# EavianWoo/SinGS

Hardware: AMD Instinct MI355X
Metric: rendered views/sec fwd+bwd, 200k Gaussians @1080p (higher is better)
Workload: dtype f32; 1 GPU; S(200000,1920,1080,deg=3,seed=3): 200000 Gaussians, 1920x1080, SH deg 3, fwd+bwd, R=780064 (tile,Gaussian) pairs, every view of a step within 0.1 % of that (cameras a few cm apart), frame-parallel dp1; gaussians=200000, width=1920, height=1080, sh_degree=3, num_rendered=780064, tile_list_max=135, frames_per_launch=8, streams=2, regularisers=False, forward_only=False, hip_graph=False, reduction=fold of 2 gradient row(s) for 16 views + collective in 1 chunk(s), gradient_rows=2, parallelism=dp1

## Files before the change

### sings_amd/_lib.py

```python
import ctypes as C
import os

_HERE = os.path.dirname(os.path.abspath(__file__))
LIB_PATH = os.environ.get("SINGS_HIP_LIB") or os.path.join(_HERE, "libsings_hip.so")
_lib = None


class SgRasterSettings(C.Structure):
    _fields_ = [
        ("image_height", C.c_int32), ("image_width", C.c_int32),
        ("tanfovx", C.c_float), ("tanfovy", C.c_float), ("scale_modifier", C.c_float),
        ("sh_degree", C.c_int32), ("sh_coeffs", C.c_int32),
        ("prefiltered", C.c_int32), ("debug", C.c_int32), ("flags", C.c_int32),
        ("bg", C.c_void_p), ("viewmatrix", C.c_void_p), ("projmatrix", C.c_void_p), ("campos", C.c_void_p),
        ("count_signal", C.c_void_p), ("count_signal_host", C.c_void_p),
    ]


class SgLayout(C.Structure):
    _fields_ = [(n, C.c_size_t) for n in (
        "geom_recA", "geom_recB", "geom_recC", "geom_depth", "geom_flags", "geom_slot", "geom_bytes",
        "bin_header", "bin_tile_count", "bin_ranges", "bin_cursor", "bin_pair_keys", "bin_point_list",
        "bin_point_keys", "bin_pair_gid", "bin_pair_tile", "bin_pair_local", "bin_sort_items", "bin_rank_items", "bin_items", "bin_ck_start", "bin_plan", "bin_pair_mask", "bin_item_w", "bin_item_perm", "bin_rec_valid", "bin_tile_keys", "bin_bytes", "img_final_T", "img_n_contrib", "img_ckpt", "img_bytes", "bwd_bytes")]


class SgSkinInputs(C.Structure):
    _fields_ = [("J", C.c_int32), ("rot_format", C.c_int32)] + [(n, C.c_void_p) for n in (
        "xyz_canon", "rot_canon", "lbs_weights", "A", "smpl_scale", "transl", "ext_trans", "ext_rot", "ext_scale")]
# ... 115 lines not shown
    "sg_mesh_midpoints_i32": "i: i3 p4",
    "sg_mesh_collapse_max_edges": "i:",
    "sg_mesh_collapse_ws_bytes": "z: i2",
    "sg_mesh_collapse_build": "i: i3 p3 d p3",
    "sg_mesh_collapse_emit": "i: i4 p6",
    "sg_init_ws_bytes": "z: i",
    "sg_init_attributes": "i: i3 f2 p12",
    "sg_attr_mse_ws_bytes": "z:",
    "sg_attr_mse": "i: i V3 p3",
    "sg_plateau_step": "i: i3 d p4 i p i p",
    "sg_profile_enable": "i: i",
    "sg_copy_probe": "i: p2 z i p",
    "sg_profile_collect": "i: d n i",
    "sg_kernel_name": "s: i",
}
_PROTOTYPES_EVAL = {
    "sg_image_metrics_ws_bytes": "z: i3",
    "sg_image_metrics_frames": "i: i4 p2 z p z p3",
}
_PROTOTYPES_MESH_TERMS = {
    "sg_mesh_terms_build": "i: i3 p13",
    "sg_mesh_terms": "i: i p4 i p13",
}
_P = C.POINTER
_CTYPE = {"i": C.c_int, "z": C.c_size_t, "f": C.c_float, "s": C.c_char_p,
          "p": C.c_void_p,
          "S": _P(SgRasterSettings), "F": _P(SgFrameBatch), "K": _P(SgSkinInputs), "L": _P(SgLayout), "T": _P(SgTriplane),
          "D": _P(SgLinearSide),
          "n": _P(C.c_int64), "Z": _P(C.c_size_t), "d": _P(C.c_double),
          "V": _P(C.c_void_p),
          "G": _P(C.c_void_p * 3 * 4)}
EXPORTS = tuple(_PROTOTYPES)
LPIPS_NUM_OFFSETS = 46
LPIPS_WS_NUM_PIECES = 28
LPIPS_MIN_SIZE = 16
NUM_KERNELS = 8
ABI_VERSION = 8
METRICS_CLAMP = 1
METRICS_FLOATS = 8
METRICS_STRIP_COLS = 64
METRICS_CHUNK_ROWS = 32
MESH_TERMS_INFO_INTS = 2
MESH_TERMS_BAD_LABEL = 1
MESH_TERMS_BAD_EDGE = 2
FLAG_SHORT_LISTS = 1
COUNT_FLAG_HALF_ROWS = 4
COUNT_FLAG_HALF_LONG_ROWS = 8
FLAG_WS_CLEAN = 2
FLAG_THROUGHPUT = 4
FLAG_FORWARD_BINNING = 8
FLAG_FORWARD_COMPOSITE = 16
FLAG_SH_PLANAR = 32
FLAG_LONG_ROWS = 64
NUM_RENDERED_LONG_LIST = -2
HDR_FLAG_OVERFLOW = 1
HDR_FLAG_LONG_LIST = 2


def _ctypes_of(signature):
    ret, _, params = signature.partition(":")
    return _CTYPE[ret], [_CTYPE[t[0]] for t in params.split() for _ in range(int(t[1:] or 1))]


def load():
    global _lib
    if _lib is not None:
        return _lib
    if not os.path.exists(LIB_PATH):
        raise RuntimeError(
            f"sings_amd: HIP library not built ({LIB_PATH} missing). There is no CPU fallback; "
            "run `make -C sings_amd/csrc` (needs hipcc, --offload-arch=gfx950).")
    import torch
    lib = C.CDLL(LIB_PATH)
    if lib.sg_abi_version() != ABI_VERSION:
        raise RuntimeError(f"sings_amd: {LIB_PATH} speaks ABI {lib.sg_abi_version()}, this host code ABI {ABI_VERSION} "
                           "(include/sings_hip.h SG_ABI_VERSION): rebuild with `make -C sings_amd/csrc`")
    for name, signature in (*_PROTOTYPES.items(), *_PROTOTYPES_EVAL.items(), *_PROTOTYPES_MESH_TERMS.items()):
        fn = getattr(lib, name)
        fn.restype, fn.argtypes = _ctypes_of(signature)
    _lib = lib
    return lib


def check(status, what):
    if status != 0:
        raise RuntimeError(f"sings_hip {what} failed: {load().sg_last_error().decode()}")


def layout(P, W, H, cap):
    L = SgLayout()
    check(load().sg_layout(P, W, H, cap, C.byref(L)), "sg_layout")
    return L


def aux_layout(P, W, H, cap):
    n = C.c_size_t(0)
    check(load().sg_aux_layout(P, W, H, cap, C.byref(n)), "sg_aux_layout")
    return int(n.value)


# ... 5 lines not shown
```

### sings_amd/csrc/sg_api_raster.hip

```cpp
#include "sg_host.h"

#include <chrono>
#include <stdlib.h>
#include <thread>

static int sg_make_cam(const SgRasterSettings *s, SgCam *c)
{
    if (!s || s->image_width <= 0 || s->image_height <= 0 || !s->viewmatrix || !s->projmatrix || !s->campos || !s->bg)
        return 1;
    if (s->sh_degree < 0 || s->sh_degree > 3) return 1;
    c->W = s->image_width; c->H = s->image_height;
    c->gx = (c->W + SG_TILE - 1) / SG_TILE; c->gy = (c->H + SG_TILE - 1) / SG_TILE;
    if ((size_t)c->gx * (size_t)c->gy >= SG_MAX_TILES) return 1;
    c->tanfovx = s->tanfovx; c->tanfovy = s->tanfovy;
    c->fx = (float)c->W / (2.0f * s->tanfovx); c->fy = (float)c->H / (2.0f * s->tanfovy);
    c->mod = s->scale_modifier; c->D = s->sh_degree; c->M = s->sh_coeffs; c->flags = s->flags;
    c->view = s->viewmatrix; c->proj = s->projmatrix; c->campos = s->campos; c->bg = s->bg;
    c->count_signal = nullptr;
    return 0;
}

static void sg_arm_count(const SgRasterSettings *s, SgCam *c, const int64_t *num_rendered_host)
{
    if (!num_rendered_host || !s->count_signal || !s->count_signal_host) return;
// ... 85 lines not shown
    hipError_t e = hipMemcpy2DAsync(r, 8, binning_ws, bin_stride ? bin_stride : 8, 8, (size_t)K, hipMemcpyDeviceToHost, (hipStream_t)stream);
    if (e == hipSuccess) e = hipStreamSynchronize((hipStream_t)stream);
    if (e != hipSuccess) return sg_set_error("sg_read_num_rendered", e);
    for (int f = 0; f < K; f++)
        num_rendered_host[f] = (r[2 * f + 1] & 2u) ? (int64_t)SG_NUM_RENDERED_LONG_LIST : (int64_t)r[2 * f];
    return 0;
}

enum SgAux { SG_AUX_NONE, SG_AUX_ONE, SG_AUX_FRAMES };

static int sg_aux_flags(const char *who, int flags, bool frames)
{
    static const struct { int bit; const char *name; } refused[] = {
        { SG_FLAG_THROUGHPUT, "SG_FLAG_THROUGHPUT" }, { SG_FLAG_FORWARD_BINNING, "SG_FLAG_FORWARD_BINNING" },
        { SG_FLAG_FORWARD_COMPOSITE, "SG_FLAG_FORWARD_COMPOSITE" }, { SG_FLAG_SH_PLANAR, "SG_FLAG_SH_PLANAR" } };
    for (const auto &r : refused)
        if ((flags & r.bit) && !(frames && r.bit == SG_FLAG_THROUGHPUT))
            return sg_failf("%s: %s is not supported with depth / alpha maps", who, r.name);
    const int known = SG_FLAG_SHORT_LISTS | SG_FLAG_LONG_ROWS | SG_FLAG_WS_CLEAN | (frames ? SG_FLAG_THROUGHPUT : 0);
    if (flags & ~known) return sg_failf("%s: unknown flags 0x%x", who, flags & ~known);
    return 0;
}

static int sg_forward_impl(const char *who, const SgRasterSettings *s, const SgFrameBatch *fb, int P, const SgSkinInputs *skin,
                           const float *means3D, const float *shs, const float *colors_precomp, const float *opacities,
                           const float *scales, const float *rotations, const float *cov3D_precomp, void *geom_ws, void *binning_ws,
                           size_t cap, void *image_ws, float *out_color, int32_t *radii, float *posed_xyz, float *posed_rotq,
                           float *posed_scales, int write_point_keys, int64_t *num_rendered_host, void *stream,
                           SgAux aux = SG_AUX_NONE, void *aux_ws = nullptr, float *out_depth = nullptr, float *out_alpha = nullptr)
{
    hipStream_t st = (hipStream_t)stream;
    SgCam c;
    if (aux && !aux_ws) return sg_failf("%s: null pointer (aux_ws)", who);
    if (sg_make_cam(s, &c)) return sg_failf("%s: bad settings", who);
    if (aux) {
        if (sg_aux_flags(who, c.flags, aux == SG_AUX_FRAMES)) return 1;
        if (!out_depth || !out_alpha) return sg_failf("%s: null pointer (out_depth / out_alpha)", who);
    }
    if (skin) {
        if (sg_check_skin(skin, P, true)) return sg_failf("%s: bad skin inputs (J in 1..64, ext_tfs all or none)", who);
        if (sg_check_placement(who, fb, skin)) return 1;
        if (P < 0 || !geom_ws || !binning_ws || !image_ws || !out_color || (P > 0 && (!shs || !opacities || !scales || !radii)))
            return sg_failf("%s: null pointer", who);
        if (s->sh_coeffs < (s->sh_degree + 1) * (s->sh_degree + 1)) return sg_failf("%s: sh_coeffs smaller than (sh_degree+1)^2", who);
    } else {
        if (sg_check_placement(who, fb, nullptr)) return 1;
        if (P < 0 || !geom_ws || !binning_ws || !image_ws || !out_color || (P > 0 && (!means3D || !opacities || !radii)))
            return sg_failf("%s: null pointer", who);
        if (P > 0 && ((shs != nullptr) == (colors_precomp != nullptr))) return sg_failf("%s: provide exactly one of shs / colors_precomp", who);
        if (P > 0 && (((scales != nullptr) && (rotations != nullptr)) == (cov3D_precomp != nullptr)))
            return sg_failf("%s: provide exactly one of (scales,rotations) / cov3D_precomp", who);
        if (shs && (s->sh_coeffs < (s->sh_degree + 1) * (s->sh_degree + 1))) return sg_failf("%s: sh_coeffs smaller than (sh_degree+1)^2", who);
    }
    SgLayout L;
    sg_layout(P, c.W, c.H, cap, &L);
    SgBatch bt;
    if (sg_make_batch(fb, P, c, L, cap, &bt)) return sg_failf("%s: bad frame batch (K in 1..16, camera_stride 0|1, transl_stride 0|3)", who);
    SgGeom g = sg_geom_view(geom_ws, L);
    SgBin b = sg_bin_view(binning_ws, L);
    SgImg im = sg_img_view(image_ws, L);
    const bool do_bin = !(c.flags & SG_FLAG_FORWARD_COMPOSITE), do_comp = !(c.flags & SG_FLAG_FORWARD_BINNING);
    if (!do_bin && !do_comp) return sg_failf("%s: SG_FLAG_FORWARD_BINNING and SG_FLAG_FORWARD_COMPOSITE exclude each other", who);
    if (do_bin) {
        if (bt.K == 1) sg_arm_count(s, &c, num_rendered_host);
        if (!(c.flags & SG_FLAG_WS_CLEAN)) {
            const size_t zb = (L.bin_tile_count - L.bin_header) + sg_ctr_count((uint32_t)c.gx, (uint32_t)c.gy) * 4;
            for (int f = 0; f < bt.K; f++) sg_zero_async((char *)b.header + (size_t)f * bt.bin, zb, st);
        }
        if (skin) sg_launch_skin_fwd(c, bt, P, skin, shs, opacities, scales, g, b, cap, radii, posed_xyz, posed_rotq, posed_scales, st);
        else sg_launch_preprocess_fwd(c, bt, P, means3D, shs, colors_precomp, opacities, scales, rotations, cov3D_precomp, g, b, cap, radii, st);
        SG_CHECK_LAST("preprocess_fwd", s, st);
        sg_launch_binning(c, bt, P, radii, g, b, cap, write_point_keys, st);
        SG_CHECK_LAST("binning", s, st);
    }
    if (do_comp) {
        SgAuxFwd ax = sg_aux_fwd_view(aux_ws, g, out_depth, out_alpha);
        ax.ws = sg_aux_bytes(cap); ax.map = (size_t)c.W * (size_t)c.H;
        sg_launch_render_fwd(c, bt, g, b, cap, im, out_color, write_point_keys, st, aux ? &ax : nullptr);
        SG_CHECK_LAST("render_fwd", s, st);
    }
    if (!do_bin) return 0;
    if (bt.K == 1) return sg_finish_count(s, c, binning_ws, num_rendered_host, stream);
    return num_rendered_host ? sg_read_counts(binning_ws, bt.bin, bt.K, num_rendered_host, stream) : 0;
}

extern "C" int sg_rasterize_forward(const SgRasterSettings *s, int P, const float *means3D, const float *shs,
                                    const float *colors_precomp, const float *opacities, const float *scales,
                                    const float *rotations, const float *cov3D_precomp, void *geom_ws,
                                    void *binning_ws, size_t cap, void *image_ws, float *out_color,
                                    int32_t *radii, int write_point_keys, int64_t *num_rendered_host, void *stream)
{
    return sg_forward_impl("sg_rasterize_forward", s, &SG_ONE_FRAME, P, nullptr, means3D, shs, colors_precomp, opacities, scales,
                           rotations, cov3D_precomp, geom_ws, binning_ws, cap, image_ws, out_color, radii, nullptr, nullptr, nullptr,
// ... 355 lines not shown
extern "C" int sg_rasterize_backward_records_frames_aux(const SgRasterSettings *s, const SgFrameBatch *fb, int P, const void *geom_ws,
                                                        const void *binning_ws, size_t cap, const void *image_ws, void *bwd_ws,
                                                        const float *dL_dout_color, void *aux_ws, const float *dL_ddepth,
                                                        const float *dL_dalpha, void *stream)
{
    return sg_records_impl("sg_rasterize_backward_records_frames_aux", s, fb, P, geom_ws, binning_ws, cap, image_ws, bwd_ws,
                           dL_dout_color, stream, SG_AUX_FRAMES, aux_ws, dL_ddepth, dL_dalpha);
}

extern "C" int sg_skinned_backward_gaussians_frames_aux(const SgRasterSettings *s, const SgFrameBatch *fb, int P, const SgSkinInputs *skin,
                                                        const float *shs, const float *opacities, const float *scales,
                                                        const int32_t *radii, const void *geom_ws, const void *binning_ws, size_t cap,
                                                        const void *bwd_ws, float *skin_ws, int accumulate,
                                                        const float *dL_dposed_xyz_in, const float *dL_dposed_rotq_in,
                                                        float *dL_dxyz_canon, float *dL_drot_canon, float *dL_dscales,
                                                        float *dL_dopacity, float *dL_dsh, float *dL_dmeans2D, float *dL_dA,
                                                        float *dL_dtransl, void *aux_ws, void *stream)
{
    (void)opacities;
    return sg_skin_gaussians_impl("sg_skinned_backward_gaussians_frames_aux", s, fb, P, skin, shs, scales, radii, geom_ws, binning_ws,
                                  cap, bwd_ws, skin_ws, accumulate, dL_dposed_xyz_in, dL_dposed_rotq_in, dL_dxyz_canon, dL_drot_canon,
                                  dL_dscales, dL_dopacity, dL_dsh, dL_dmeans2D, dL_dA, dL_dtransl, stream, SG_AUX_FRAMES, aux_ws);
}
```

### sings_amd/csrc/sg_host.h

```cpp
#pragma once
#include "sg_common.h"

#include <math.h>
#include <stdarg.h>
#include <stdio.h>

static inline int sg_failf(const char *fmt, ...)
{
    char msg[256];
    va_list ap;
    va_start(ap, fmt);
    vsnprintf(msg, sizeof msg, fmt, ap);
    va_end(ap);
    return sg_set_error(msg, hipSuccess);
}

static inline int sg_launched(const char *what)
{
    const hipError_t e = hipGetLastError();
    return e == hipSuccess ? 0 : sg_set_error(what, e);
}

static inline void sg_ssim_window(float w[11])
{
    float g[11];
    double s = 0.0;
    for (int x = 0; x < 11; x++) { g[x] = (float)exp(-(double)((x - 5) * (x - 5)) / (2.0 * 1.5 * 1.5)); s += (double)g[x]; }
    for (int x = 0; x < 11; x++) w[x] = g[x] / (float)s;
}

#define SG_CHECK_LAST(what, s, st)                                           \
    do {                                                                     \
        hipError_t e_ = hipGetLastError();                                   \
        if (e_ != hipSuccess) return sg_set_error(what, e_);                 \
        if ((s)->debug) {                                                    \
            e_ = hipStreamSynchronize(st);                                   \
            if (e_ != hipSuccess) return sg_set_error(what, e_);             \
        }                                                                    \
    } while (0)

int sg_launch_linear_bwd_fan(int N, int Cin, int Cout, int act, const float *z, const float *dh, const float *W, float *dz_out,
                             float *dx_out, const SgLinearSide *side, hipStream_t st);
void sg_launch_scales_head(int N, const float *z, float *scales, float *aux, const float *dscales, const float *daux, float *dz,
                           hipStream_t st);
void sg_launch_rows_laplacian(int R, int V, int C, const float *x, const int *row_ptr, const int *col, const float *val,
                              const float *rscale, const int *t_row_ptr, const int *t_row, const float *t_val, void *ws, float *g_ws,
                              float *loss, const float *upstream, float *dL_dx, hipStream_t st);
```

### sings_amd/csrc/sg_preprocess.hip

```cpp
#include "sg_project.h"

template <int D>
__global__ void __launch_bounds__(256)
sg_preprocess_fwd_kernel(SgCam c, SgBatch bt, int P, const float *__restrict__ means3D,
                         const float *__restrict__ shs, const float *__restrict__ colors_precomp,
                         const float *__restrict__ opacities, const float *__restrict__ scales,
                         const float *__restrict__ rotations, const float *__restrict__ cov3D_precomp,
                         SgGeom g, SgBin bn, uint32_t cap, int32_t *__restrict__ radii, int hist_tiles, int nblocks)
{
    extern __shared__ uint32_t sg_hist_lds[];
    __shared__ uint32_t scratch_all[4][256];
    int gblock, frame;
    if (!sg_block_frame((int)blockIdx.x, bt.K, nblocks, gblock, frame)) return;
    c = sg_frame(c, frame, bt.cam_stride); g = sg_frame(g, (size_t)frame * bt.geom); bn = sg_frame(bn, (size_t)frame * bt.bin);
    radii += (size_t)frame * bt.P;
    const int idx = gblock * 256 + (int)threadIdx.x;
    const int wave = threadIdx.x >> 6;
    const bool live = idx < P;
    constexpr int nc = (D + 1) * (D + 1);
    float sh[nc * 3];
    if (shs && live) {
        const float *src = shs + (size_t)idx * c.M * 3;
        if (D == 3 && c.M == 16) {
#pragma unroll
            for (int k = 0; k < nc * 3 / 4; k++) {
                const float4 v = ((const float4 *)src)[k];
                sh[4 * k] = v.x; sh[4 * k + 1] = v.y; sh[4 * k + 2] = v.z; sh[4 * k + 3] = v.w;
            }
        } else {
#pragma unroll
            for (int k = 0; k < nc * 3; k++) sh[k] = src[k];
        }
    }
    SgProj o;
    o.mr = 0; o.tt = 0; o.clampbits = 0; o.x0 = o.y0 = o.x1 = o.y1 = 0;
    o.pix[0] = o.pix[1] = 0; o.conic[0] = o.conic[1] = o.conic[2] = 0; o.rgb[0] = o.rgb[1] = o.rgb[2] = 0; o.depth = 0;
    float opac = 0.0f;
    if (live) {
        float p[3] = { means3D[3 * idx], means3D[3 * idx + 1], means3D[3 * idx + 2] };
        float s3[3] = { 0, 0, 0 }, q[4] = { 0, 0, 0, 0 };
        if (!cov3D_precomp) {
            s3[0] = scales[3 * idx]; s3[1] = scales[3 * idx + 1]; s3[2] = scales[3 * idx + 2];
            q[0] = rotations[4 * idx]; q[1] = rotations[4 * idx + 1]; q[2] = rotations[4 * idx + 2]; q[3] = rotations[4 * idx + 3];
        }
        sg_project_fwd<D>(c, p, s3, q, cov3D_precomp ? cov3D_precomp + 6 * (size_t)idx : nullptr,
                          colors_precomp ? colors_precomp + 3 * (size_t)idx : nullptr, sh, o);
        opac = opacities[idx];
    }
    sg_store_proj(live, idx, o, opac, g, bn, c.gx, cap, radii, scratch_all[wave], hist_tiles ? sg_hist_lds : nullptr, hist_tiles,
                  sg_key_pitch_of(hist_tiles != 0, c.flags));
}

void sg_launch_preprocess_fwd(const SgCam &c, const SgBatch &bt, int P, const float *means3D, const float *shs,
                              const float *colors_precomp, const float *opacities, const float *scales,
                              const float *rotations, const float *cov3D_precomp, SgGeom g, SgBin b,
                              size_t cap, int32_t *radii, hipStream_t st)
{
    if (P <= 0) return;
    const int nblocks = (P + 255) / 256;
    dim3 grid(sg_frame_grid(nblocks, bt.K)), block(256);
    const int ht = sg_lds_hist(c.gx, c.gy) ? (int)sg_ctr_count((uint32_t)c.gx, (uint32_t)c.gy) : 0;
#define SG_PP(DD) hipLaunchKernelGGL(sg_preprocess_fwd_kernel<DD>, grid, block, (size_t)ht * 4, st, c, bt, P, means3D, shs, \
                                     colors_precomp, opacities, scales, rotations, cov3D_precomp, g, b, sg_cap32(cap), radii, ht, nblocks)
    int D = colors_precomp ? 0 : c.D;
    sg_prof_begin(SG_K_PREPROCESS_FWD, st);
    switch (D) { case 0: SG_PP(0); break; case 1: SG_PP(1); break; case 2: SG_PP(2); break; default: SG_PP(3); break; }
    sg_prof_end(SG_K_PREPROCESS_FWD, st);
#undef SG_PP
}

#define SG_PBWD_PARAMS SgCam c, int P, const float *__restrict__ means3D, const float *__restrict__ shs,                              \
                       const float *__restrict__ colors_precomp, const float *__restrict__ scales,                                \
                       const float *__restrict__ rotations, const float *__restrict__ cov3D_precomp,                              \
                       const int32_t *__restrict__ radii, SgGeom g, SgRec grec,                                                   \
                       size_t cap, const uint32_t *__restrict__ header, const uint8_t *__restrict__ rec_valid, float *__restrict__ dL_dmeans3D, float *__restrict__ dL_dmeans2D, \
                       float *__restrict__ dL_dsh, float *__restrict__ dL_dcolors,                                                \
                       float *__restrict__ dL_dopacity, float *__restrict__ dL_dscales,                                           \
                       float *__restrict__ dL_drots, float *__restrict__ dL_dcov3D
#define SG_PBWD_AUX 0
#include "sg_preprocess_bwd.inc"
#undef SG_PBWD_AUX
#define SG_PBWD_AUX 1
#include "sg_preprocess_bwd.inc"
#undef SG_PBWD_AUX

#define SG_ACC_PITCH 257
template <int D, bool ACC>
__global__ void __launch_bounds__(256) __attribute__((amdgpu_waves_per_eu(2, D >= 2 ? 2 : 3)))
sg_preprocess_bwd_frames_kernel(SgCam c0, SgBatch bt, int P, const float *__restrict__ means3D, const float *__restrict__ shs,
                         const float *__restrict__ colors_precomp, const float *__restrict__ scales,
                         const float *__restrict__ rotations, const float *__restrict__ cov3D_precomp,
// ... 231 lines not shown
```

### sings_amd/csrc/sg_project.h

```cpp
#pragma once
#include "sg_math.h"

template <int D>
__device__ __forceinline__ void sg_eval_sh(const float *__restrict__ sh, const float dir[3],
                                           float rgb[3], uint32_t &clampbits)
{
    float b[16];
    sg_sh_basis<D>(dir, b);
    constexpr int nc = (D + 1) * (D + 1);
    clampbits = 0;
#pragma unroll
    for (int c = 0; c < 3; c++) {
        float acc = b[0] * sh[c];
#pragma unroll
        for (int k = 1; k < nc; k++) acc = acc + b[k] * sh[3 * k + c];
        acc = acc + 0.5f;
        if (acc < 0.0f) { clampbits |= 1u << c; acc = 0.0f; }
        rgb[c] = acc;
    }
}


struct SgProj {
    int mr;
// ... 178 lines not shown
        }
    }
    if (expand) {
#pragma unroll
        for (int u = 0; u < 4; u++) {
            const uint32_t p = 64 * u + lane;
            const uint32_t slot = base + p;
            if (direct) {
                if (p < total) {
                    const uint32_t rank = local0[u] + (hist ? hist[ctr0[u]] : 0u);
                    if (rank < key_pitch) SG_KEY_STORE(&bn.tile_keys[(size_t)tile0[u] * key_pitch + rank], ((uint64_t)dep0[u] << 32) | gj0[u]);
                    else bn.header[8] = 1u;
                    if (hist && slot < cap) bn.rec_valid[slot] = 0;
                }
            } else if (p < total && slot < cap) {
                bn.pair_gid[slot] = gj0[u]; bn.pair_tile[slot] = tile0[u];
                bn.pair_local[slot] = local0[u] + (hist ? hist[ctr0[u]] : 0u);
            }
        }
    }
    __builtin_amdgcn_wave_barrier();
}

#define SG_ROW_LDS 52
__device__ __forceinline__ void sg_rows48_load(const float *__restrict__ base, int g0, int P, int lane,
                                               float *__restrict__ l)
{
    const float4 *src = (const float4 *)(base + (size_t)g0 * 48);
    const int nf4 = (P - g0 < 64 ? P - g0 : 64) * 12;
#pragma unroll
    for (int i = 0; i < 12; i++) {
        const int f = i * 64 + lane;
        if (f < nf4) {
            const float4 v = src[f];
            const int row = f / 12, c4 = f - row * 12;
            *(float4 *)(l + row * SG_ROW_LDS + 4 * c4) = v;
        }
    }
}
__device__ __forceinline__ void sg_rows48_store(float *__restrict__ base, int g0, int P, int lane,
                                                const float *__restrict__ l, int rows = 64, bool accumulate = false)
{
    float4 *dst = (float4 *)(base + (size_t)g0 * 48);
    const int nf4 = (P - g0 < rows ? (P - g0 > 0 ? P - g0 : 0) : rows) * 12;
    if (accumulate) {
        float4 old[12];
// ... 290 lines not shown
```

### sings_amd/engine.py

```python
import ctypes as C

import torch

from . import _lib
from ._marshal import _camera_stride, _frame_batch, _frame_rows, _ptr, _settings_struct, _skin_frames, _skin_struct
from ._marshal import _stream as _current_stream


def _raster_fields(M):
    return [("d_means3D", 3), ("d_scales", 3), ("d_rots", 4), ("d_opacity", 1), ("d_sh", 3 * M if M else None)]


def _skinned_fields(M, with_rot, rot_width):
    return [("d_xyz", 3), ("d_scales", 3), ("d_opacity", 1), ("d_sh", 3 * M), ("d_rot", int(rot_width) if with_rot else None)]


class _Engine:

    def __init__(self, P, W, H, sh_coeffs, device, capacity_pairs, K=None):
        self.lib = _lib.load()
        if K is not None and not 1 <= K <= _lib.MAX_FRAMES:
            raise ValueError(f"K must be 1..{_lib.MAX_FRAMES}")
        self.P, self.W, self.H, self.M, self.cap = int(P), int(W), int(H), int(sh_coeffs), int(capacity_pairs)
        self.K = 1 if K is None else int(K)
        self.dev = torch.device(device)
        L = _lib.SgLayout()
        sizes = [C.c_size_t() for _ in range(4)]
        _lib.check(self.lib.sg_frames_layout(self.P, self.W, self.H, self.cap, self.K, C.byref(L), *[C.byref(x) for x in sizes]),
                   "sg_frames_layout")
# ... 355 lines not shown
                       "skinned backward (records, frames, depth / alpha maps)")
        else:
            _lib.check(self.lib.sg_rasterize_backward_records_frames(*args, self._stream()), "skinned backward (records, frames)")

    def backward_gaussians(self, shs, opacities, scales, accumulate=False):
        self._check_backward()
        accumulate, done = self._chain_begin(accumulate)
        if self.aux and accumulate:
            raise ValueError("SkinnedFramesEngine: the depth / alpha maps (aux=True) write the gradients (no accumulate)")
        args = (C.byref(self._s), C.byref(self._fb), self.P, C.byref(self._k), _ptr(shs), _ptr(opacities), _ptr(scales),
                _ptr(self.radii), _ptr(self.geom), _ptr(self.binning), self.cap, _ptr(self.bwd_ws), _ptr(self.skin_ws),
                int(accumulate), None, None, _ptr(self.d_xyz), _ptr(self.d_rot), _ptr(self.d_scales), _ptr(self.d_opacity),
                _ptr(self.d_sh), _ptr(self.d_means2D), _ptr(self.d_A), _ptr(self.d_transl))
        if self.aux:
            _lib.check(self.lib.sg_skinned_backward_gaussians_frames_aux(*args, _ptr(self.aux_ws), self._stream()),
                       "skinned backward (gaussians, frames, depth / alpha maps)")
        else:
            _lib.check(self.lib.sg_skinned_backward_gaussians_frames(*args, self._stream()), "skinned backward (gaussians, frames)")
        self._chain_end(done)


class RasterFramesEngine(_FramesEngine):

    def __init__(self, P, W, H, sh_coeffs, K, device, capacity_pairs, grad_flat=None, sh_planar=False):
        super().__init__(P, W, H, sh_coeffs, device, capacity_pairs, K)
        self._gradients(_raster_fields(self.M), grad_flat, sh_planar)

    def set_camera(self, raster_settings, short_lists=False, long_rows=False):
        self._camera(raster_settings, (_lib.FLAG_SHORT_LISTS if short_lists else 0) | (_lib.FLAG_LONG_ROWS if long_rows else 0))
        self._fb = _frame_batch(self.K, self._cam_stride, 0)

    def forward(self, means3D, shs, opacities, scales, rotations, sync_num_rendered=False):
        if self._s is None or self._fb is None:
            raise RuntimeError("RasterFramesEngine: set_camera() first")
        nr = (C.c_int64 * self.K)()
        self._s.flags = self._flags()
        self._clean = False
        _lib.check(self.lib.sg_rasterize_forward_frames(
            C.byref(self._s), C.byref(self._fb), self.P, _ptr(means3D), _ptr(shs), None, _ptr(opacities), _ptr(scales),
            _ptr(rotations), None, _ptr(self.geom), _ptr(self.binning), self.cap, _ptr(self.img), _ptr(self.color),
            _ptr(self.radii), nr if sync_num_rendered else None, self._stream()), "forward (frames)")
        self._clean = True
        return [int(v) for v in nr] if sync_num_rendered else None

    def backward(self, means3D, shs, opacities, scales, rotations, dL_dcolor, accumulate=False):
        _lib.check(self.lib.sg_rasterize_backward_records_frames(
            C.byref(self._s), C.byref(self._fb), self.P, _ptr(self.geom), _ptr(self.binning), self.cap, _ptr(self.img),
            _ptr(self.bwd_ws), _ptr(dL_dcolor), self._stream()), "backward (records, frames)")
        accumulate, done = self._chain_begin(accumulate)
        _lib.check(self.lib.sg_rasterize_backward_gaussians_frames(
            C.byref(self._s), C.byref(self._fb), self.P, _ptr(means3D), _ptr(shs), None, _ptr(opacities), _ptr(scales),
            _ptr(rotations), None, _ptr(self.radii), _ptr(self.geom), _ptr(self.binning), self.cap, _ptr(self.bwd_ws),
            int(accumulate), _ptr(self.d_means3D), _ptr(self.d_means2D), _ptr(self.d_sh), None, _ptr(self.d_opacity),
            _ptr(self.d_scales), _ptr(self.d_rots), None, self._stream()), "backward (gaussians, frames)")
        self._chain_end(done)


class FramePipeline:

    def __init__(self, engines, device):
        self.engines = list(engines)
        self.dev = torch.device(device)
        self.A = torch.cuda.Stream(self.dev)
        self.B = torch.cuda.Stream(self.dev, priority=-1)
# ... 35 lines not shown
```

Baseline: 5473 views/s.

## Bin Gaussians in Morton work order with windowed LDS tile counting

Computes 3D Morton codes of the Gaussian means on the GPU, sorts them once into a work order, and splits forward preprocessing into a no-binning projection kernel plus an ordered binning kernel. The binning kernel visits Gaussians in spatial order so each block's tile footprint is compact and can be counted in an LDS window before global atomics. The goal is fewer contended global atomics on tile counters when the per-tile histogram does not fit in LDS. It costs an extra kernel launch and an order built once and cached, which can go stale as the Gaussians move.

```diff
diff --git a/include/sings_order.h b/include/sings_order.h
--- /dev/null
+++ b/include/sings_order.h
@@ -0,0 +1,26 @@
+#ifndef SINGS_ORDER_H
+#define SINGS_ORDER_H
+
+#include "sings_hip.h"
+
+#ifdef __cplusplus
+extern "C" {
+#endif
+
+#define SG_ORDER_WINDOW_TILES 1536
+#define SG_ORDER_BLOCK 256
+#define SG_ORDER_CODE_BITS 10
+#define SG_ORDER_WS_BYTES 32
+
+int sg_rasterize_forward_frames_ordered(const SgRasterSettings *s, const SgFrameBatch *fb, int P, const float *means3D,
+                                        const float *shs, const float *colors_precomp, const float *opacities,
+                                        const float *scales, const float *rotations, const float *cov3D_precomp, void *geom_ws,
+                                        void *binning_ws, size_t cap, void *image_ws, float *out_color, int32_t *radii,
+                                        int64_t *num_rendered_host, const uint32_t *order, int order_len, void *stream);
+
+int sg_work_order_codes(int P, const float *means3D, void *ws, uint32_t *codes, void *stream);
+
+#ifdef __cplusplus
+}
+#endif
+#endif
diff --git a/sings_amd/_lib.py b/sings_amd/_lib.py
--- a/sings_amd/_lib.py
+++ b/sings_amd/_lib.py
@@ -4,6 +4,7 @@
 _HERE = os.path.dirname(os.path.abspath(__file__))
 LIB_PATH = os.environ.get("SINGS_HIP_LIB") or os.path.join(_HERE, "libsings_hip.so")
 _lib = None
+HAS_ORDER = False
 
 
 class SgRasterSettings(C.Structure):
@@ -165,6 +166,10 @@
     "sg_mesh_terms_build": "i: i3 p13",
     "sg_mesh_terms": "i: i p4 i p13",
 }
+_PROTOTYPES_ORDER = {
+    "sg_rasterize_forward_frames_ordered": "i: S F i p9 z p3 n p i p",
+    "sg_work_order_codes": "i: i p4",
+}
 _P = C.POINTER
 _CTYPE = {"i": C.c_int, "z": C.c_size_t, "f": C.c_float, "s": C.c_char_p,
           "p": C.c_void_p,
@@ -183,6 +188,11 @@
 METRICS_FLOATS = 8
 METRICS_STRIP_COLS = 64
 METRICS_CHUNK_ROWS = 32
+ORDER_WINDOW_TILES = 1536
+ORDER_BLOCK = 256
+ORDER_CODE_BITS = 10
+ORDER_WS_BYTES = 32
+HIST_TILES_MAX = 4096
 MESH_TERMS_INFO_INTS = 2
 MESH_TERMS_BAD_LABEL = 1
 MESH_TERMS_BAD_EDGE = 2
@@ -218,7 +228,12 @@
     if lib.sg_abi_version() != ABI_VERSION:
         raise RuntimeError(f"sings_amd: {LIB_PATH} speaks ABI {lib.sg_abi_version()}, this host code ABI {ABI_VERSION} "
                            "(include/sings_hip.h SG_ABI_VERSION): rebuild with `make -C sings_amd/csrc`")
-    for name, signature in (*_PROTOTYPES.items(), *_PROTOTYPES_EVAL.items(), *_PROTOTYPES_MESH_TERMS.items()):
+    global HAS_ORDER
+    HAS_ORDER = all(hasattr(lib, name) for name in _PROTOTYPES_ORDER)
+    if not HAS_ORDER and LIB_PATH == os.path.join(_HERE, "libsings_hip.so"):
+        raise RuntimeError(f"sings_amd: {LIB_PATH} lacks the entry points of include/sings_order.h: rebuild with `make -C sings_amd/csrc`")
+    for name, signature in (*_PROTOTYPES.items(), *_PROTOTYPES_EVAL.items(), *_PROTOTYPES_MESH_TERMS.items(),
+                            *(_PROTOTYPES_ORDER.items() if HAS_ORDER else ())):
         fn = getattr(lib, name)
         fn.restype, fn.argtypes = _ctypes_of(signature)
     _lib = lib
diff --git a/sings_amd/csrc/sg_api_raster.hip b/sings_amd/csrc/sg_api_raster.hip
--- a/sings_amd/csrc/sg_api_raster.hip
+++ b/sings_amd/csrc/sg_api_raster.hip
@@ -1,4 +1,5 @@
 #include "sg_host.h"
+#include "../../include/sings_order.h"
 
 #include <chrono>
 #include <stdlib.h>
@@ -131,15 +132,24 @@
     return 0;
 }
 
+static int sg_check_order(const char *who, const uint32_t *order, int order_len, int P)
+{
+    if (!order) return order_len ? sg_failf("%s: order_len %d without an order", who, order_len) : 0;
+    if (order_len != P) return sg_failf("%s: the order has %d entries, the call %d Gaussians", who, order_len, P);
+    return 0;
+}
+
 static int sg_forward_impl(const char *who, const SgRasterSettings *s, const SgFrameBatch *fb, int P, const SgSkinInputs *skin,
                            const float *means3D, const float *shs, const float *colors_precomp, const float *opacities,
                            const float *scales, const float *rotations, const float *cov3D_precomp, void *geom_ws, void *binning_ws,
                            size_t cap, void *image_ws, float *out_color, int32_t *radii, float *posed_xyz, float *posed_rotq,
                            float *posed_scales, int write_point_keys, int64_t *num_rendered_host, void *stream,
-                           SgAux aux = SG_AUX_NONE, void *aux_ws = nullptr, float *out_depth = nullptr, float *out_alpha = nullptr)
+                           SgAux aux = SG_AUX_NONE, void *aux_ws = nullptr, float *out_depth = nullptr, float *out_alpha = nullptr,
+                           const uint32_t *order = nullptr, int order_len = 0)
 {
     hipStream_t st = (hipStream_t)stream;
     SgCam c;
+    if (sg_check_order(who, order, order_len, P)) return 1;
     if (aux && !aux_ws) return sg_failf("%s: null pointer (aux_ws)", who);
     if (sg_make_cam(s, &c)) return sg_failf("%s: bad settings", who);
     if (aux) {
@@ -177,7 +187,8 @@
             for (int f = 0; f < bt.K; f++) sg_zero_async((char *)b.header + (size_t)f * bt.bin, zb, st);
         }
         if (skin) sg_launch_skin_fwd(c, bt, P, skin, shs, opacities, scales, g, b, cap, radii, posed_xyz, posed_rotq, posed_scales, st);
-        else sg_launch_preprocess_fwd(c, bt, P, means3D, shs, colors_precomp, opacities, scales, rotations, cov3D_precomp, g, b, cap, radii, st);
+        else sg_launch_preprocess_fwd_ordered(c, bt, P, means3D, shs, colors_precomp, opacities, scales, rotations, cov3D_precomp, g, b, cap,
+                                              radii, order, st);
         SG_CHECK_LAST("preprocess_fwd", s, st);
         sg_launch_binning(c, bt, P, radii, g, b, cap, write_point_keys, st);
         SG_CHECK_LAST("binning", s, st);
@@ -579,3 +590,24 @@
                                   cap, bwd_ws, skin_ws, accumulate, dL_dposed_xyz_in, dL_dposed_rotq_in, dL_dxyz_canon, dL_drot_canon,
                                   dL_dscales, dL_dopacity, dL_dsh, dL_dmeans2D, dL_dA, dL_dtransl, stream, SG_AUX_FRAMES, aux_ws);
 }
+
+extern "C" int sg_rasterize_forward_frames_ordered(const SgRasterSettings *s, const SgFrameBatch *fb, int P, const float *means3D,
+                                                   const float *shs, const float *colors_precomp, const float *opacities,
+                                                   const float *scales, const float *rotations, const float *cov3D_precomp,
+                                                   void *geom_ws, void *binning_ws, size_t cap, void *image_ws, float *out_color,
+                                                   int32_t *radii, int64_t *num_rendered_host, const uint32_t *order, int order_len,
+                                                   void *stream)
+{
+    return sg_forward_impl("sg_rasterize_forward_frames_ordered", s, fb, P, nullptr, means3D, shs, colors_precomp, opacities, scales,
+                           rotations, cov3D_precomp, geom_ws, binning_ws, cap, image_ws, out_color, radii, nullptr, nullptr, nullptr,
+                           0, num_rendered_host, stream, SG_AUX_NONE, nullptr, nullptr, nullptr, order, order_len);
+}
+
+extern "C" int sg_work_order_codes(int P, const float *means3D, void *ws, uint32_t *codes, void *stream)
+{
+    if (P < 0) return sg_failf("sg_work_order_codes: P = %d", P);
+    if (P == 0) return 0;
+    if (!means3D || !ws || !codes) return sg_failf("sg_work_order_codes: null pointer");
+    sg_launch_morton_codes(P, means3D, (float *)ws, codes, (hipStream_t)stream);
+    return sg_launched("sg_work_order_codes");
+}
diff --git a/sings_amd/csrc/sg_host.h b/sings_amd/csrc/sg_host.h
--- a/sings_amd/csrc/sg_host.h
+++ b/sings_amd/csrc/sg_host.h
@@ -46,3 +46,10 @@
 void sg_launch_rows_laplacian(int R, int V, int C, const float *x, const int *row_ptr, const int *col, const float *val,
                               const float *rscale, const int *t_row_ptr, const int *t_row, const float *t_val, void *ws, float *g_ws,
                               float *loss, const float *upstream, float *dL_dx, hipStream_t st);
+
+static inline bool sg_order_applies(const SgCam &c) { return !sg_lds_hist(c.gx, c.gy) && sg_key_pitch_of(false, c.flags) != 0u; }
+void sg_launch_preprocess_fwd_ordered(const SgCam &c, const SgBatch &bt, int P, const float *means3D, const float *shs,
+                                      const float *colors_precomp, const float *opacities, const float *scales,
+                                      const float *rotations, const float *cov3D_precomp, SgGeom g, SgBin b,
+                                      size_t cap, int32_t *radii, const uint32_t *order, hipStream_t st);
+void sg_launch_morton_codes(int P, const float *means3D, float *box, uint32_t *codes, hipStream_t st);
diff --git a/sings_amd/csrc/sg_order.hip b/sings_amd/csrc/sg_order.hip
--- /dev/null
+++ b/sings_amd/csrc/sg_order.hip
@@ -0,0 +1,65 @@
+#include "sg_host.h"
+#include "../../include/sings_order.h"
+
+__global__ void __launch_bounds__(1024)
+sg_order_box_kernel(int P, const float *__restrict__ means3D, float *__restrict__ box)
+{
+    __shared__ float sLo[3][1024 / SG_WAVE], sHi[3][1024 / SG_WAVE];
+    float lo[3] = { INFINITY, INFINITY, INFINITY }, hi[3] = { -INFINITY, -INFINITY, -INFINITY };
+    for (int i = threadIdx.x; i < P; i += 1024)
+#pragma unroll
+        for (int k = 0; k < 3; k++) {
+            const float v = means3D[3 * (size_t)i + k];
+            lo[k] = fminf(lo[k], v); hi[k] = fmaxf(hi[k], v);
+        }
+    const int lane = threadIdx.x & 63, wave = threadIdx.x >> 6;
+#pragma unroll
+    for (int k = 0; k < 3; k++) {
+#pragma unroll
+        for (int s = 32; s > 0; s >>= 1) {
+            lo[k] = fminf(lo[k], __shfl_xor(lo[k], s, 64));
+            hi[k] = fmaxf(hi[k], __shfl_xor(hi[k], s, 64));
+        }
+        if (lane == 0) { sLo[k][wave] = lo[k]; sHi[k][wave] = hi[k]; }
+    }
+    __syncthreads();
+    if (threadIdx.x < 3) {
+        const int k = threadIdx.x;
+        float a = sLo[k][0], b = sHi[k][0];
+        for (int w = 1; w < 1024 / SG_WAVE; w++) { a = fminf(a, sLo[k][w]); b = fmaxf(b, sHi[k][w]); }
+        box[k] = a; box[3 + k] = b;
+    }
+}
+
+__device__ __forceinline__ uint32_t sg_spread10(uint32_t v)
+{
+    v &= 0x3ffu;
+    v = (v | (v << 16)) & 0x030000ffu;
+    v = (v | (v << 8)) & 0x0300f00fu;
+    v = (v | (v << 4)) & 0x030c30c3u;
+    v = (v | (v << 2)) & 0x09249249u;
+    return v;
+}
+
+__global__ void __launch_bounds__(256)
+sg_order_codes_kernel(int P, const float *__restrict__ means3D, const float *__restrict__ box, uint32_t *__restrict__ codes)
+{
+    const int i = blockIdx.x * 256 + threadIdx.x;
+    if (i >= P) return;
+    uint32_t code = 0;
+#pragma unroll
+    for (int k = 0; k < 3; k++) {
+        const float lo = box[k], ext = fmaxf(box[3 + k] - lo, 1e-12f);
+        const float q = (means3D[3 * (size_t)i + k] - lo) * (1023.0f / ext);
+        const uint32_t cell = q >= 1023.0f ? 1023u : q > 0.0f ? (uint32_t)q : 0u;
+        code |= sg_spread10(cell) << k;
+    }
+    codes[i] = code;
+}
+
+void sg_launch_morton_codes(int P, const float *means3D, float *box, uint32_t *codes, hipStream_t st)
+{
+    if (P <= 0) return;
+    hipLaunchKernelGGL(sg_order_box_kernel, dim3(1), dim3(1024), 0, st, P, means3D, box);
+    hipLaunchKernelGGL(sg_order_codes_kernel, dim3((P + 255) / 256), dim3(256), 0, st, P, means3D, box, codes);
+}
diff --git a/sings_amd/csrc/sg_preprocess.hip b/sings_amd/csrc/sg_preprocess.hip
--- a/sings_amd/csrc/sg_preprocess.hip
+++ b/sings_amd/csrc/sg_preprocess.hip
@@ -1,6 +1,7 @@
 #include "sg_project.h"
-
-template <int D>
+#include "sg_host.h"
+
+template <int D, bool NOBIN>
 __global__ void __launch_bounds__(256)
 sg_preprocess_fwd_kernel(SgCam c, SgBatch bt, int P, const float *__restrict__ means3D,
                          const float *__restrict__ shs, const float *__restrict__ colors_precomp,
@@ -9,7 +10,7 @@
                          SgGeom g, SgBin bn, uint32_t cap, int32_t *__restrict__ radii, int hist_tiles, int nblocks)
 {
     extern __shared__ uint32_t sg_hist_lds[];
-    __shared__ uint32_t scratch_all[4][256];
+    __shared__ uint32_t scratch_all[4][NOBIN ? 1 : 256];
     int gblock, frame;
     if (!sg_block_frame((int)blockIdx.x, bt.K, nblocks, gblock, frame)) return;
     c = sg_frame(c, frame, bt.cam_stride); g = sg_frame(g, (size_t)frame * bt.geom); bn = sg_frame(bn, (size_t)frame * bt.bin);
@@ -47,8 +48,28 @@
                           colors_precomp ? colors_precomp + 3 * (size_t)idx : nullptr, sh, o);
         opac = opacities[idx];
     }
+    if constexpr (NOBIN)
+        sg_store_proj_nobin(live, idx, o, opac, g, bn, radii);
+    else
     sg_store_proj(live, idx, o, opac, g, bn, c.gx, cap, radii, scratch_all[wave], hist_tiles ? sg_hist_lds : nullptr, hist_tiles,
                   sg_key_pitch_of(hist_tiles != 0, c.flags));
+}
+
+__global__ void __launch_bounds__(256)
+sg_bin_ordered_kernel(SgBatch bt, int P, SgGeom g, SgBin bn, int gx, uint32_t key_pitch, const uint32_t *__restrict__ order)
+{
+    __shared__ uint32_t scratch_all[4][320];
+    const int frame = blockIdx.y;
+    g = sg_frame(g, (size_t)frame * bt.geom); bn = sg_frame(bn, (size_t)frame * bt.bin);
+    const int pos = blockIdx.x * 256 + (int)threadIdx.x, wave = threadIdx.x >> 6;
+    uint32_t gid = pos < P ? order[pos] : 0xffffffffu;
+    uint32_t rmin = 0u, rwh = 0u, dep = 0u;
+    if (gid < (uint32_t)P) {
+        const float4 rc = g.recC[SG_REC_STRIDE * (size_t)gid];
+        rmin = __float_as_uint(rc.z); rwh = __float_as_uint(rc.w);
+        dep = __float_as_uint(g.depth[gid]);
+    } else gid = 0u;
+    sg_bin_ordered(gid, rmin, rwh, dep, bn, gx, scratch_all[wave], scratch_all[wave] + 256, key_pitch);
 }
 
 void sg_launch_preprocess_fwd(const SgCam &c, const SgBatch &bt, int P, const float *means3D, const float *shs,
@@ -56,17 +77,31 @@
                               const float *rotations, const float *cov3D_precomp, SgGeom g, SgBin b,
                               size_t cap, int32_t *radii, hipStream_t st)
 {
+    sg_launch_preprocess_fwd_ordered(c, bt, P, means3D, shs, colors_precomp, opacities, scales, rotations, cov3D_precomp, g, b, cap,
+                                     radii, nullptr, st);
+}
+
+void sg_launch_preprocess_fwd_ordered(const SgCam &c, const SgBatch &bt, int P, const float *means3D, const float *shs,
+                                      const float *colors_precomp, const float *opacities, const float *scales,
+                                      const float *rotations, const float *cov3D_precomp, SgGeom g, SgBin b,
+                                      size_t cap, int32_t *radii, const uint32_t *order, hipStream_t st)
+{
     if (P <= 0) return;
     const int nblocks = (P + 255) / 256;
     dim3 grid(sg_frame_grid(nblocks, bt.K)), block(256);
     const int ht = sg_lds_hist(c.gx, c.gy) ? (int)sg_ctr_count((uint32_t)c.gx, (uint32_t)c.gy) : 0;
-#define SG_PP(DD) hipLaunchKernelGGL(sg_preprocess_fwd_kernel<DD>, grid, block, (size_t)ht * 4, st, c, bt, P, means3D, shs, \
+    const bool ord = order && sg_order_applies(c);
+#define SG_PPO(DD, OO) hipLaunchKernelGGL((sg_preprocess_fwd_kernel<DD, OO>), grid, block, (size_t)ht * 4, st, c, bt, P, means3D, shs, \
                                      colors_precomp, opacities, scales, rotations, cov3D_precomp, g, b, sg_cap32(cap), radii, ht, nblocks)
+#define SG_PP(DD) do { if (ord) SG_PPO(DD, true); else SG_PPO(DD, false); } while (0)
     int D = colors_precomp ? 0 : c.D;
     sg_prof_begin(SG_K_PREPROCESS_FWD, st);
     switch (D) { case 0: SG_PP(0); break; case 1: SG_PP(1); break; case 2: SG_PP(2); break; default: SG_PP(3); break; }
+    if (ord)
+        hipLaunchKernelGGL(sg_bin_ordered_kernel, dim3(nblocks, bt.K), block, 0, st, bt, P, g, b, c.gx, sg_key_pitch_of(false, c.flags), order);
     sg_prof_end(SG_K_PREPROCESS_FWD, st);
 #undef SG_PP
+#undef SG_PPO
 }
 
 #define SG_PBWD_PARAMS SgCam c, int P, const float *__restrict__ means3D, const float *__restrict__ shs,                              \
diff --git a/sings_amd/csrc/sg_project.h b/sings_amd/csrc/sg_project.h
--- a/sings_amd/csrc/sg_project.h
+++ b/sings_amd/csrc/sg_project.h
@@ -1,5 +1,6 @@
 #pragma once
 #include "sg_math.h"
+#include "../../include/sings_order.h"
 
 template <int D>
 __device__ __forceinline__ void sg_eval_sh(const float *__restrict__ sh, const float dir[3],
@@ -224,6 +225,169 @@
     __builtin_amdgcn_wave_barrier();
 }
 
+__device__ __forceinline__ void sg_store_proj_nobin(bool live, int idx, const SgProj &o, float opac, SgGeom g, SgBin bn,
+                                                    int32_t *__restrict__ radii)
+{
+    __shared__ uint32_t sWaveTot[4];
+    __shared__ uint32_t sBlockBase;
+    const int lane = threadIdx.x & 63, wave_ = (threadIdx.x >> 6) & 3;
+    uint32_t incl = o.tt;
+#pragma unroll
+    for (int s = 1; s < 64; s <<= 1) {
+        uint32_t v = __shfl_up(incl, s, 64);
+        if (lane >= s) incl += v;
+    }
+    if (lane == 63) sWaveTot[wave_] = incl;
+    const uint32_t rmin = (uint32_t)o.x0 | ((uint32_t)o.y0 << 16);
+    const uint32_t rwh = (uint32_t)(o.x1 - o.x0) | ((uint32_t)(o.y1 - o.y0) << 16);
+    if (live) {
+        radii[idx] = o.mr;
+        g.recA[SG_REC_STRIDE * (size_t)idx] = make_float4(o.pix[0], o.pix[1], o.conic[0], o.conic[1]);
+        g.recB[SG_REC_STRIDE * (size_t)idx] = make_float4(o.conic[2], o.mr ? opac : 0.0f, o.rgb[0], o.rgb[1]);
+        g.depth[idx] = o.depth;
+        g.flags[idx] = o.clampbits;
+    }
+    __syncthreads();
+    if (threadIdx.x == 0) {
+        uint32_t t = sWaveTot[0] + sWaveTot[1] + sWaveTot[2] + sWaveTot[3];
+        sBlockBase = t ? atomicAdd(&bn.header[2], t) : 0u;
+    }
+    __syncthreads();
+    uint32_t base = sBlockBase;
+    for (int w = 0; w < wave_; w++) base += sWaveTot[w];
+    if (live) {
+        g.recC[SG_REC_STRIDE * (size_t)idx] = make_float4(o.rgb[2], __uint_as_float(base + incl - o.tt), __uint_as_float(rmin), __uint_as_float(rwh));
+        g.slot[idx] = make_uint2(base + incl - o.tt, rwh);
+    }
+}
+
+#define SG_ORDER_WINDOW_MAX SG_ORDER_WINDOW_TILES
+__device__ __forceinline__ void sg_bin_ordered(uint32_t gid, uint32_t rmin, uint32_t rwh, uint32_t depthbits, SgBin bn, int gx,
+                                               uint32_t *__restrict__ scratch, uint32_t *__restrict__ sGid, uint32_t key_pitch)
+{
+    uint32_t *sIncl = scratch, *sMin = scratch + 64, *sWid = scratch + 128, *sDep = scratch + 192;
+    __shared__ uint32_t sWindow[SG_ORDER_WINDOW_MAX];
+    __shared__ uint32_t sWaveWin[4][4];
+    const int lane = threadIdx.x & 63, wave_ = (threadIdx.x >> 6) & 3;
+    const uint32_t rw = rwh & 0xffffu, rh = rwh >> 16, tt = rw * rh;
+    uint32_t incl = tt;
+#pragma unroll
+    for (int s = 1; s < 64; s <<= 1) {
+        uint32_t v = __shfl_up(incl, s, 64);
+        if (lane >= s) incl += v;
+    }
+    const uint32_t total = __shfl(incl, 63, 64);
+    uint32_t wx0 = tt ? (rmin & 0xffffu) : 0xffffu, wy0 = tt ? (rmin >> 16) : 0xffffu;
+    uint32_t wx1 = tt ? (rmin & 0xffffu) + rw : 0u, wy1 = tt ? (rmin >> 16) + rh : 0u;
+#pragma unroll
+    for (int s = 32; s > 0; s >>= 1) {
+        const uint32_t a = __shfl_xor(wx0, s, 64), b = __shfl_xor(wy0, s, 64), c = __shfl_xor(wx1, s, 64), d = __shfl_xor(wy1, s, 64);
+        wx0 = a < wx0 ? a : wx0; wy0 = b < wy0 ? b : wy0; wx1 = c > wx1 ? c : wx1; wy1 = d > wy1 ? d : wy1;
+    }
+    if (lane == 63) { sWaveWin[wave_][0] = wx0; sWaveWin[wave_][1] = wy0; sWaveWin[wave_][2] = wx1; sWaveWin[wave_][3] = wy1; }
+    for (int t = threadIdx.x; t < SG_ORDER_WINDOW_MAX; t += 256) sWindow[t] = 0u;
+    sIncl[lane] = incl; sMin[lane] = rmin; sWid[lane] = rw; sDep[lane] = depthbits; sGid[lane] = gid;
+    __syncthreads();
+    uint32_t X0 = sWaveWin[0][0], Y0 = sWaveWin[0][1], X1 = sWaveWin[0][2], Y1 = sWaveWin[0][3];
+#pragma unroll
+    for (int w = 1; w < 4; w++) {
+        X0 = sWaveWin[w][0] < X0 ? sWaveWin[w][0] : X0; Y0 = sWaveWin[w][1] < Y0 ? sWaveWin[w][1] : Y0;
+        X1 = sWaveWin[w][2] > X1 ? sWaveWin[w][2] : X1; Y1 = sWaveWin[w][3] > Y1 ? sWaveWin[w][3] : Y1;
+    }
+    const bool any = X1 > X0 && Y1 > Y0;
+    if (!any) return;
+    const uint32_t ww = X1 - X0, wh = Y1 - Y0;
+    const bool windowed = ww * wh <= (uint32_t)SG_ORDER_WINDOW_MAX;
+    uint32_t tile[4], gj[4], dep[4], cell[4];
+    auto expand = [&](uint32_t p0) {
+#pragma unroll
+        for (int u = 0; u < 4; u++) {
+            const uint32_t p = p0 + 64 * u + lane;
+            tile[u] = 0; gj[u] = 0; dep[u] = 0; cell[u] = 0;
+            if (p < total) {
+                int lo = 0, hi = 63;
+#pragma unroll
+                for (int it = 0; it < 6; it++) {
+                    int mid = (lo + hi) >> 1;
+                    if (sIncl[mid] > p) hi = mid; else lo = mid + 1;
+                }
+                const int j = lo;
+                const uint32_t excl = j ? sIncl[j - 1] : 0u;
+                const uint32_t t = p - excl, w = sWid[j], mn = sMin[j];
+                const uint32_t ty = (uint32_t)(((float)t + 0.5f) / (float)w);
+                const uint32_t tx = t - ty * w;
+                const uint32_t ax = (mn & 0xffffu) + tx, ay = (mn >> 16) + ty;
+                tile[u] = ay * (uint32_t)gx + ax;
+                gj[u] = sGid[j];
+                dep[u] = sDep[j];
+                cell[u] = windowed ? (ay - Y0) * ww + (ax - X0) : sg_ctr_index(ax, ay, (uint32_t)gx);
+            }
+        }
+    };
+    auto store_key = [&](uint32_t tl, uint32_t rank, uint32_t d, uint32_t gi) {
+        if (rank < key_pitch) SG_KEY_STORE(&bn.tile_keys[(size_t)tl * key_pitch + rank], ((uint64_t)d << 32) | gi);
+        else bn.header[8] = 1u;
+    };
+    if (!windowed) {
+        for (uint32_t p0 = 0; p0 < total; p0 += 256) {
+            expand(p0);
+            uint32_t rank[4];
+#pragma unroll
+            for (int u = 0; u < 4; u++) rank[u] = p0 + 64 * u + lane < total ? atomicAdd(&bn.tile_count[cell[u]], 1u) : 0u;
+#pragma unroll
+            for (int u = 0; u < 4; u++)
+                if (p0 + 64 * u + lane < total) store_key(tile[u], rank[u], dep[u], gj[u]);
+        }
+        return;
+    }
+    uint32_t tile0[4], gj0[4], dep0[4], cell0[4];
+    expand(0u);
+#pragma unroll
+    for (int u = 0; u < 4; u++) {
+        tile0[u] = tile[u]; gj0[u] = gj[u]; dep0[u] = dep[u]; cell0[u] = cell[u];
+        if (64 * u + lane < total) atomicAdd(&sWindow[cell[u]], 1u);
+    }
+    for (uint32_t p0 = 256; p0 < total; p0 += 256) {
+        expand(p0);
+#pragma unroll
+        for (int u = 0; u < 4; u++)
+            if (p0 + 64 * u + lane < total) atomicAdd(&sWindow[cell[u]], 1u);
+    }
+    __syncthreads();
+    {
+        const uint32_t bx0 = X0 >> 2, by0 = Y0 >> 2, bxn = ((X1 - 1u) >> 2) - bx0 + 1u, byn = ((Y1 - 1u) >> 2) - by0 + 1u;
+        const uint32_t cover = bxn * byn * 16u, cbx = sg_ctr_blocks_x((uint32_t)gx);
+        for (uint32_t c0 = threadIdx.x; c0 < cover; c0 += 4 * 256) {
+            uint32_t cnt[4], lc[4], ctr[4], ans[4];
+#pragma unroll
+            for (int u = 0; u < 4; u++) {
+                const uint32_t c = c0 + 256u * u, b = c >> 4, i = c & 15u;
+                const uint32_t bby = (uint32_t)(((float)b + 0.5f) / (float)bxn), bbx = b - bby * bxn;
+                const uint32_t ax = ((bx0 + bbx) << 2) + (i & 3u), ay = ((by0 + bby) << 2) + (i >> 2);
+                const bool in = c < cover && ax >= X0 && ax < X1 && ay >= Y0 && ay < Y1;
+                lc[u] = in ? (ay - Y0) * ww + (ax - X0) : 0u;
+                ctr[u] = ((by0 + bby) * cbx + bx0 + bbx) * 16u + i;
+                cnt[u] = in ? sWindow[lc[u]] : 0u;
+            }
+#pragma unroll
+            for (int u = 0; u < 4; u++) ans[u] = cnt[u] ? atomicAdd(&bn.tile_count[ctr[u]], cnt[u]) : 0u;
+#pragma unroll
+            for (int u = 0; u < 4; u++)
+                if (cnt[u]) sWindow[lc[u]] = ans[u];
+        }
+    }
+    __syncthreads();
+#pragma unroll
+    for (int u = 0; u < 4; u++)
+        if (64 * u + lane < total) store_key(tile0[u], atomicAdd(&sWindow[cell0[u]], 1u), dep0[u], gj0[u]);
+    for (uint32_t p0 = 256; p0 < total; p0 += 256) {
+        expand(p0);
+#pragma unroll
+        for (int u = 0; u < 4; u++)
+            if (p0 + 64 * u + lane < total) store_key(tile[u], atomicAdd(&sWindow[cell[u]], 1u), dep[u], gj[u]);
+    }
+}
+
 #define SG_ROW_LDS 52
 __device__ __forceinline__ void sg_rows48_load(const float *__restrict__ base, int g0, int P, int lane,
                                                float *__restrict__ l)
diff --git a/sings_amd/engine.py b/sings_amd/engine.py
--- a/sings_amd/engine.py
+++ b/sings_amd/engine.py
@@ -1,10 +1,15 @@
 import ctypes as C
+import os
 
 import torch
 
 from . import _lib
+from . import work_order as _work_order
 from ._marshal import _camera_stride, _frame_batch, _frame_rows, _ptr, _settings_struct, _skin_frames, _skin_struct
 from ._marshal import _stream as _current_stream
+
+
+_ORDER_BY_DEFAULT = os.environ.get("SINGS_WORK_ORDER", "1") != "0"
 
 
 def _raster_fields(M):
@@ -406,24 +411,51 @@
 
 class RasterFramesEngine(_FramesEngine):
 
-    def __init__(self, P, W, H, sh_coeffs, K, device, capacity_pairs, grad_flat=None, sh_planar=False):
+    def __init__(self, P, W, H, sh_coeffs, K, device, capacity_pairs, grad_flat=None, sh_planar=False, order=None):
         super().__init__(P, W, H, sh_coeffs, device, capacity_pairs, K)
         self._gradients(_raster_fields(self.M), grad_flat, sh_planar)
+        self.set_order(order)
+
+    def set_order(self, order):
+        if order is None and not _ORDER_BY_DEFAULT:
+            order = False
+        self._order_auto = order is None
+        self._order = None if order is None or order is False else _work_order.check_order(order, self.P, self.geom.device)
 
     def set_camera(self, raster_settings, short_lists=False, long_rows=False):
         self._camera(raster_settings, (_lib.FLAG_SHORT_LISTS if short_lists else 0) | (_lib.FLAG_LONG_ROWS if long_rows else 0))
         self._fb = _frame_batch(self.K, self._cam_stride, 0)
 
+    def refresh_order(self):
+        if self._order_auto:
+            self._order = None
+
+    def _order_for(self, means3D):
+        if self._order is not None and not _lib.HAS_ORDER:
+            raise RuntimeError("RasterFramesEngine: this library predates include/sings_order.h and takes no work order")
+        if (self._order is None and self._order_auto and _lib.HAS_ORDER and self.P > 0
+                and _work_order.order_applies(self.W, self.H, self._rows)):
+            if torch.cuda.is_current_stream_capturing():
+                raise RuntimeError("RasterFramesEngine: the work order is built on the first forward, which cannot be inside a graph "
+                                   "capture (run one forward first, or pass order=False / order=<tensor>)")
+            self._order = _work_order.build_order(means3D)
+        return self._order
+
     def forward(self, means3D, shs, opacities, scales, rotations, sync_num_rendered=False):
         if self._s is None or self._fb is None:
             raise RuntimeError("RasterFramesEngine: set_camera() first")
+        order = self._order_for(means3D)
         nr = (C.c_int64 * self.K)()
         self._s.flags = self._flags()
         self._clean = False
-        _lib.check(self.lib.sg_rasterize_forward_frames(
-            C.byref(self._s), C.byref(self._fb), self.P, _ptr(means3D), _ptr(shs), None, _ptr(opacities), _ptr(scales),
-            _ptr(rotations), None, _ptr(self.geom), _ptr(self.binning), self.cap, _ptr(self.img), _ptr(self.color),
-            _ptr(self.radii), nr if sync_num_rendered else None, self._stream()), "forward (frames)")
+        args = (C.byref(self._s), C.byref(self._fb), self.P, _ptr(means3D), _ptr(shs), None, _ptr(opacities), _ptr(scales),
+                _ptr(rotations), None, _ptr(self.geom), _ptr(self.binning), self.cap, _ptr(self.img), _ptr(self.color),
+                _ptr(self.radii), nr if sync_num_rendered else None)
+        if order is None:
+            _lib.check(self.lib.sg_rasterize_forward_frames(*args, self._stream()), "forward (frames)")
+        else:
+            _lib.check(self.lib.sg_rasterize_forward_frames_ordered(*args, _ptr(order), order.numel(), self._stream()),
+                       "forward (frames, ordered)")
         self._clean = True
         return [int(v) for v in nr] if sync_num_rendered else None
 
diff --git a/sings_amd/work_order.py b/sings_amd/work_order.py
--- /dev/null
+++ b/sings_amd/work_order.py
@@ -0,0 +1,78 @@
+import ctypes as C
+
+import numpy as np
+
+from . import _lib
+
+
+def morton_codes_host(xyz):
+    x = np.ascontiguousarray(xyz, dtype=np.float32).reshape(-1, 3)
+    if x.shape[0] == 0:
+        return np.zeros(0, np.uint32)
+    with np.errstate(all="ignore"):
+        lo, hi = np.fmin.reduce(x, axis=0), np.fmax.reduce(x, axis=0)
+        ext = np.fmax(hi - lo, np.float32(1e-12)).astype(np.float32)
+        q = (x - lo).astype(np.float32) * (np.float32(1023.0) / ext).astype(np.float32)
+        cell = np.where(q >= np.float32(1023.0), np.float32(1023.0), np.where(q > 0, q, np.float32(0))).astype(np.uint32)
+    code = np.zeros(x.shape[0], np.uint32)
+    for k in range(3):
+        for b in range(_lib.ORDER_CODE_BITS):
+            code |= ((cell[:, k] >> np.uint32(b)) & np.uint32(1)) << np.uint32(3 * b + k)
+    return code
+
+
+def order_host(xyz):
+    return np.argsort(morton_codes_host(xyz), kind="stable").astype(np.int32)
+
+
+def build_order(means3D):
+    import torch
+    from ._marshal import _ptr, _stream
+    if means3D.dtype != torch.float32 or means3D.dim() != 2 or means3D.shape[1] != 3 or not means3D.is_cuda:
+        raise ValueError("build_order: means3D must be an fp32 [P,3] tensor on the GPU")
+    m = means3D.detach().contiguous()
+    P = m.shape[0]
+    codes = torch.empty(P, dtype=torch.int32, device=m.device)
+    ws = torch.empty(_lib.ORDER_WS_BYTES, dtype=torch.uint8, device=m.device)
+    _lib.check(_lib.load().sg_work_order_codes(P, _ptr(m), C.c_void_p(ws.data_ptr()), _ptr(codes), _stream(m.device)),
+               "sg_work_order_codes")
+    return torch.sort(codes, stable=True)[1].to(torch.int32)
+
+
+def check_order(order, P, device):
+    import torch
+    if not torch.is_tensor(order) or order.dtype != torch.int32 or order.dim() != 1 or not order.is_contiguous():
+        raise ValueError("order must be a contiguous int32 tensor [P]")
+    if order.numel() != P:
+        raise ValueError(f"order has {order.numel()} entries, the engine {P} Gaussians")
+    if order.device != device:
+        raise ValueError(f"order is on {order.device}, the engine on {device}")
+    return order
+
+
+def order_applies(W, H, flags):
+    gx, gy = (W + 15) // 16, (H + 15) // 16
+    return bool(flags & _lib.FLAG_SHORT_LISTS) and ((gx + 3) // 4) * ((gy + 3) // 4) * 16 > _lib.HIST_TILES_MAX
+
+
+def window_census(rect_min, rect_max, order=None):
+    mn, mx = np.asarray(rect_min, np.int64), np.asarray(rect_max, np.int64)
+    if order is not None:
+        o = np.asarray(order, np.int64)
+        mn, mx = mn[o], mx[o]
+    P, B = mn.shape[0], _lib.ORDER_BLOCK
+    w, h = np.maximum(mx[:, 0] - mn[:, 0], 0), np.maximum(mx[:, 1] - mn[:, 1], 0)
+    area = w * h
+    pairs, group_tiles, windows = int(area.sum()), 0, []
+    for b0 in range(0, P, B):
+        sel = np.nonzero(area[b0:b0 + B])[0] + b0
+        if sel.size == 0:
+            windows.append(0)
+            continue
+        x0, y0, x1, y1 = mn[sel, 0].min(), mn[sel, 1].min(), mx[sel, 0].max(), mx[sel, 1].max()
+        windows.append(int((x1 - x0) * (y1 - y0)))
+        seen = np.zeros((y1 - y0, x1 - x0), bool)
+        for i in sel:
+            seen[mn[i, 1] - y0:mx[i, 1] - y0, mn[i, 0] - x0:mx[i, 0] - x0] = True
+        group_tiles += int(seen.sum())
+    return {"pairs": pairs, "group_tiles": group_tiles, "windows": np.asarray(windows, np.int64)}
```

Result: faster. 5622 views/s, median of 6 (+2.7%).
